# andrewhou1/GeomConsistentFR

Measured on AMD Instinct MI355X. Metric: ray_steps_per_sec, higher is better.
Workload: dtype f64+f32

## Files before the change

### geomconsistentfr_amd/_lib.py

```python
import ctypes
import os

import torch

from . import build as _build

_LIB = None

GCFR_OK = 0
ABI_VERSION = 6
_ERRORS = {-1: "GCFR_ERR_INVALID_ARGUMENT", -2: "GCFR_ERR_LAUNCH"}

_p, _i, _f, _d = ctypes.c_void_p, ctypes.c_int32, ctypes.c_float, ctypes.c_double

N_COUNTERS = 28
COUNTER_NAMES = ("tiles", "groups_nominal", "groups_visited", "bound_tests", "bodies", "lane_samples", "early_exits",
                 "tie_remarches", "samples_in_range", "bounds_given_up", "visits_after_last_body", "visits_before_first_body",
                 "trail_enter", "trail_skips", "trail_leave", "rough_samples", "wave_samples", "wave_samples_taken", "lane_takes",
                 "audit_bound_checks", "audit_bound_violations", "audit_term_checks", "audit_term_violations",
                 "audit_masked_checks", "audit_masked_violations", "audit_safe_violations", "audit_max_use")


class Options(ctypes.Structure):
    _fields_ = [("struct_size", ctypes.c_uint32), ("tile_w", _i), ("group", _i), ("ksplit", _i),
                ("depth_bound_skip", _i), ("lds_stage", _i),
                ("event_start", _p), ("event_stop", _p), ("counters", _p), ("pixels", _i), ("phase", _i)]


def options(tile_w=0, group=0, ksplit=-1, depth_bound_skip=-1, event_start=None,
            event_stop=None, counters=None, lds_stage=-1, pixels=0, phase=0) -> Options:
    o = Options()
    load().gcfr_options_default(ctypes.byref(o))
    o.tile_w, o.group, o.ksplit, o.depth_bound_skip = tile_w, group, ksplit, depth_bound_skip
    o.lds_stage = lds_stage
    o.event_start, o.event_stop, o.counters = event_start, event_stop, counters
    o.pixels = pixels
    o.phase = phase
    return o


def _with(o, field: str, value: int) -> Options:
    n = Options()
    if o is None:
        load().gcfr_options_default(ctypes.byref(n))
    else:
        ctypes.memmove(ctypes.byref(n), ctypes.byref(o), ctypes.sizeof(Options))
    setattr(n, field, value)
    return n


def with_phase(o, phase: int) -> Options:
    return _with(o, "phase", phase)


def with_pixels(o, pixels: int) -> Options:
    return _with(o, "pixels", pixels)


def opt_ref(o):
    return ctypes.byref(o) if o is not None else None


_SIGNATURES = {
    "gcfr_version": (ctypes.c_char_p, []),
    "gcfr_abi_version": (_i, []),
    "gcfr_sample_table": (_i, [_d, _d, _i, _p]),
    "gcfr_light_prep": (_i, [_p, _i, _i, _f, _f, _p, _p, _p]),
    "gcfr_shadow_workspace_bytes": (ctypes.c_size_t, [_i, _i, _i]),
    "gcfr_options_default": (None, [_p]),
    "gcfr_render_from_depth_fwd": (_i, [_p, _i, _f, _f, _p, _p, _i, _d, _d, _d, _d, _f, _i, _p, _p, _i, _i, _i, _i, _i, _p,
                                        _f, _p, _f, _p, _p, _p, _p, _p, _p, _p, _p, _p, _p, ctypes.c_size_t, _p, _p]),
    "gcfr_normals_fwd": (_i, [_p, _i, _i, _i, _d, _d, _d, _d, _f, _i, _p, _p]),
    "gcfr_normals_bwd": (_i, [_p, _p, _i, _i, _i, _d, _d, _d, _d, _f, _i, _p, _p]),
    "gcfr_render_fwd": (_i, [_p, _i, _f, _f, _p, _p, _i, _p, _p, _p, _i, _i, _i, _i, _i, _p, _f, _p, _f,
                             _p, _p, _p, _p, _p, _p, _p, _p, _p, ctypes.c_size_t, _p, _p]),
    "gcfr_shadow_fwd": (_i, [_p, _p, _i, _p, _i, _i, _i, _i, _i, _p, _f, _p, _p, _p, _p, ctypes.c_size_t, _p, _p]),
    "gcfr_shade_fwd": (_i, [_p, _p, _p, _p, _p, _p, _i, _i, _i, _i, _f, _p, _p, _p, _p, _p]),
    "gcfr_shadow_bwd": (_i, [_p, _p, _p, _p, _i, _i, _i, _i, _i, _p, _p, _p, _p]),
    "gcfr_shade_bwd": (_i, [_p, _p, _p, _p, _p, _p, _i, _i, _i, _i, _f, _p, _p, _p, _p, _p, _p, _p, _p, _p, _p, _p]),
    "gcfr_render_bwd": (_i, [_p, _p, _p, _p, _p, _p, _p, _i, _i, _i, _i, _i, _p, _d, _d, _d, _d, _f, _i, _f, _p, _p, _p, _p, _p,
                             _p, _p, _p, _p, _p]),
    "gcfr_light_prep_bwd": (_i, [_p, _i, _i, _f, _f, _p, _p, _p, _p]),
    "gcfr_inference_images_u8": (_i, [_p, _p, _p, _p, _p, _p, _p, _p, _p, _i, _i, _i, _i, _i, _p, _p, _p, _p, _p, _p, _i, _p]),
    "gcfr_fix_border_u8": (_i, [_p, _p, _i, _i, _i, _i, _p, _p]),
    "gcfr_assemble_batch_u8": (_i, [_p, _p, _p, _p, _i, _i, _i, _p, _p, _p, _p, _p]),
    "gcfr_masked_metrics_workspace_bytes": (ctypes.c_size_t, [_i, _i, _i]),
    "gcfr_masked_metrics_u8": (_i, [_p, _p, _p, _i, _i, _i, _i, _p, _p, _p, ctypes.c_size_t, _p]),
    "gcfr_image_losses_workspace_bytes": (ctypes.c_size_t, [_i, _i, _i]),
    "gcfr_image_losses_fwd": (_i, [_p, _p, _p, _i, _i, _i, _i, _p, _d, _p, _p, _p, _p, ctypes.c_size_t, _p]),
    "gcfr_image_losses_bwd": (_i, [_p, _p, _p, _i, _i, _i, _i, _p, _d, _p, _p, _p, _p, _p]),
    "gcfr_supervised_losses_workspace_bytes": (ctypes.c_size_t, [_i, _i, _i]),
    "gcfr_supervised_losses_fwd": (_i, [_p, _p, _p, _p, _p, _p, _p, _p, _p, _p, ctypes.c_int64, _i, _i, _i, _p, _p, _p, ctypes.c_size_t, _p]),
    "gcfr_supervised_losses_bwd": (_i, [_p, _p, _p, _p, _p, _p, _p, _p, _p, ctypes.c_int64, _i, _i, _i, _p, _p, _p, _p, _p, _p, _p, _p,
                                        _p, _p, _p, _p]),
    "gcfr_light_rig_fwd": (_i, [_p, _p, _p, _i, _i, _i, _i, _i, _p, _p, _p]),
    "gcfr_light_rig_bwd": (_i, [_p, _p, _p, _i, _i, _i, _i, _i, _p, _p, _p, _p, _p, _p]),
    "gcfr_light_rig_frames_u8": (_i, [_p, _p, _p, _p, _i, _i, _p, _i, _i, _i, _i, _i, _i, _p, _p]),
    "gcfr_ingest_photographs_u8": (_i, [_p, _i, _i, _i, _i, _p, _p]),
    "gcfr_fullres_composites_u8": (_i, [_p, _p, _p, _p, _i, _i, _i, _i, _i, _i, _f, _f, _p, _p]),
    "gcfr_fullres_composites_guided_u8": (_i, [_p, _p, _p, _p, _i, _i, _i, _i, _i, _i, _f, _f, _f, _p, _p]),
    "gcfr_ingest_box_u8": (_i, [_p, _i, _i, _i, _p, _i, _i, _p, _p]),
    "gcfr_fullres_composites_box_u8": (_i, [_p, _p, _p, _p, _i, _i, _i, _i, _i, _p, _i, _i, _i, _f, _f, _p, _p]),
    "gcfr_fullres_composites_box_guided_u8": (_i, [_p, _p, _p, _p, _i, _i, _i, _i, _i, _p, _i, _i, _i, _f, _f, _f, _p, _p]),
# ... 153 lines not shown
```

### geomconsistentfr_amd/csrc/gcfr_march.hpp

```cpp
#pragma once

#include "gcfr_device.hpp"
#include "gcfr_mutants.hpp"

#include "../../include/gcfr.h"

#include <atomic>
#include <cstddef>
#include <type_traits>

namespace gcfr {

struct ShadowArgs {
    const float *depth;
    const uint8_t *mask;
    const float *light_pt;
    const double *t_table;
    float *min_dist;
    int32_t *argmin;
    int32_t mask_batch, L, H, W, N;
    int32_t tiles_x, tiles_per_image;
    float bonus, bx_lo, bx_hi, by_lo, by_hi;
};

// ... 132 lines not shown
}
__device__ inline float lane_value(float v, int lane)
{
    return __builtin_bit_cast(float, __builtin_amdgcn_readlane(__builtin_bit_cast(int, v), lane));
}


constexpr int kQueueSlot = 64;
enum { kTfOk = 0, kTfStride = 1, kTfTabs = 2, kTfTfirst = 3, kTfInvDt = 4 };
constexpr int kStatChunk = 16384;
__host__ __device__ inline int stat_chunk_shift(int H, int W)
{
    const int raw = (H * W + kStatChunk - 1) >> 14;
    return (raw > 8 && raw <= 16) ? 15 : 14;
}
__host__ __device__ inline int stat_chunk_px(int H, int W) { return 1 << stat_chunk_shift(H, W); }
__host__ __device__ inline int n_stat_chunks(int H, int W)
{
    const int sh = stat_chunk_shift(H, W);
    return (H * W + (1 << sh) - 1) >> sh;
}
static_assert(kStatChunk == 1 << 14, "stat_chunk_shift() spells kStatChunk as a shift");


struct MarchEpilogueArgs {
    float *min_dist;
    int32_t *argmin;
    float bonus, bx_lo, bx_hi, by_lo, by_hi;
    const float *normals;
    const float *albedo;
    const float *ambient;
    float *shadow_w, *full, *final_shading, *rendered;
    float intensity;
    NormalsArgs nrm;
    float *normals_out;
};

struct ShadowQuadArgs {
    const float *depth;
    const float4 *quad;
    const int *bbox;
    const int *diag;
    const float4 *zb;
    const int *zrange;
    const int *mones;
    int *tflag;
    const uint8_t *mask;
    const uint32_t *reserved0;
    const float *light_pt;
    const double *t_table;
    unsigned long long *counters;
    int32_t mask_batch, B, L, H, W, N;
    int32_t tiles_x, tiles_y;
    int32_t bl_offset;
    int32_t hz_off;
    MarchEpilogueArgs epi;
};

typedef const __attribute__((address_space(4))) ShadowQuadArgs *ArgPtr;
typedef const __attribute__((address_space(4))) MarchEpilogueArgs *EpiPtr;
__device__ __forceinline__ ArgPtr kernel_args()
{
    return (ArgPtr)__builtin_amdgcn_kernarg_segment_ptr();
}
template <class T>
__device__ __forceinline__ T launder(T p)
{
    asm volatile("" : "+s"(p));
    return p;
}

constexpr double kRintMagic = 6755399441055744.0;
typedef float f32x4 __attribute__((ext_vector_type(4)));

__device__ inline int lo32(double v)
{
    return (int)(unsigned)(__builtin_bit_cast(unsigned long long, v) & 0xffffffffull);
}

enum { kCntTiles, kCntGroupsNominal, kCntGroupsVisited, kCntBoundTests, kCntBodies, kCntLaneSamples, kCntEarlyExit,
       kCntTieRemarch, kCntSamplesInRange, kCntBoundsGivenUp, kCntVisitsAfterLastBody, kCntVisitsBeforeFirstBody,
       kCntTrailEnter, kCntTrailSkips, kCntTrailLeave, kCntRoughSamples, kCntWaveSamples, kCntWaveSamplesTaken, kCntLaneTakes,
       kCntAuditBoundChecks, kCntAuditBoundViol, kCntAuditTermChecks, kCntAuditTermViol, kCntAuditMaskedChecks, kCntAuditMaskedViol,
       kCntAuditSafeViol, kCntAuditMaxUse, kCntUsed };
static_assert(kCntUsed <= GCFR_N_COUNTERS, "gcfr_options.counters holds GCFR_N_COUNTERS tallies");
#if defined(GCFR_AUDIT) && !defined(GCFR_COUNTERS)
#error "-DGCFR_AUDIT needs -DGCFR_COUNTERS"
#endif
#ifdef GCFR_COUNTERS
#define GCFR_COUNT(i, n) (cnt[i] += (unsigned)(n))
#else
#define GCFR_COUNT(i, n) ((void)0)
#endif

struct ImageStats {
    int r_min, c_min, r_max, c_max;
    int s_min, s_max, d_min, d_max;
    int gz_lo_s, gz_nhi_s;
    int mask_all_ones;
};
__device__ inline ImageStats reduce_image_stats(ArgPtr a, int b, int lane, bool want_z)
{
    const int n = n_stat_chunks(a->H, a->W);
    if (n <= 8) {
        typedef const __attribute__((address_space(4))) int *ConstI32Ptr;
        const ConstI32Ptr sb = (ConstI32Ptr)(unsigned long long)a->bbox + 4 * (size_t)(a->mask_batch == 1 ? 0 : b) * n;
        const ConstI32Ptr sz = (ConstI32Ptr)(unsigned long long)a->zrange + 2 * (size_t)b * n;
        const ConstI32Ptr so = (ConstI32Ptr)(unsigned long long)a->mones + (size_t)(a->mask_batch == 1 ? 0 : b) * n;
        const ConstI32Ptr sd = (ConstI32Ptr)(unsigned long long)a->diag + 4 * (size_t)(a->mask_batch == 1 ? 0 : b) * n;
        int d0 = kBBoxInit, d1 = kBBoxInit, d2 = kBBoxInit, d3 = kBBoxInit;
        int m0 = kBBoxInit, m1 = kBBoxInit, m2 = kBBoxInit, m3 = kBBoxInit, z0 = 0x7fffffff, z1 = 0x7fffffff, ones = 1;
#pragma unroll
        for (int j = 0; j < 8; ++j) {
            if (j < n) {
                m0 = min(m0, sb[4 * j + 0]);
                m1 = min(m1, sb[4 * j + 1]);
                m2 = min(m2, sb[4 * j + 2]);
                m3 = min(m3, sb[4 * j + 3]);
                ones = min(ones, so[j]);
                d0 = min(d0, sd[4 * j + 0]);
                d1 = min(d1, sd[4 * j + 1]);
                d2 = min(d2, sd[4 * j + 2]);
                d3 = min(d3, sd[4 * j + 3]);
                if (want_z) {
                    z0 = min(z0, sz[2 * j + 0]);
                    z1 = min(z1, sz[2 * j + 1]);
                }
            }
        }
        ImageStats st;
        st.r_min = m0;
        st.c_min = m1;
        st.r_max = -m2;
        st.c_max = -m3;
        st.gz_lo_s = z0;
        st.gz_nhi_s = z1;
        st.mask_all_ones = ones;
        st.s_min = d0;
        st.s_max = -d1;
        st.d_min = d2;
        st.d_max = -d3;
        return st;
    }
    const int4 *pb = (const int4 *)a->bbox + (size_t)(a->mask_batch == 1 ? 0 : b) * n;
    const int2 *pz = (const int2 *)a->zrange + (size_t)b * n;
    const int *po = a->mones + (size_t)(a->mask_batch == 1 ? 0 : b) * n;
    const int4 *pd = (const int4 *)a->diag + (size_t)(a->mask_batch == 1 ? 0 : b) * n;
    int4 m = make_int4(kBBoxInit, kBBoxInit, kBBoxInit, kBBoxInit), dg = m;
    int2 mz = make_int2(0x7fffffff, 0x7fffffff);
    int ones = 1;
    for (int j = lane; j < n; j += 64) {
        ones = min(ones, po[j]);
        const int4 v = pb[j];
        m.x = min(m.x, v.x);
        m.y = min(m.y, v.y);
        m.z = min(m.z, v.z);
        m.w = min(m.w, v.w);
        const int4 w = pd[j];
        dg.x = min(dg.x, w.x);
        dg.y = min(dg.y, w.y);
        dg.z = min(dg.z, w.z);
        dg.w = min(dg.w, w.w);
        if (want_z) {
            const int2 vz = pz[j];
            mz.x = min(mz.x, vz.x);
            mz.y = min(mz.y, vz.y);
        }
    }
    ImageStats st;
    st.r_min = wave_min_i32(m.x);
    st.c_min = wave_min_i32(m.y);
    st.r_max = -wave_min_i32(m.z);
    st.c_max = -wave_min_i32(m.w);
    st.gz_lo_s = want_z ? wave_min_i32(mz.x) : 0x7fffffff;
    st.gz_nhi_s = want_z ? wave_min_i32(mz.y) : 0x7fffffff;
    st.mask_all_ones = wave_min_i32(ones);
    st.s_min = wave_min_i32(dg.x);
    st.s_max = -wave_min_i32(dg.y);
    st.d_min = wave_min_i32(dg.z);
    st.d_max = -wave_min_i32(dg.w);
    return st;
}

__device__ inline int fresh_lane_id()
{
    int l;
    asm volatile("v_mbcnt_lo_u32_b32 %0, -1, 0\n\tv_mbcnt_hi_u32_b32 %0, -1, %0" : "=v"(l));
    return l;
}

enum { kModeInline = 0, kModeFull = 1, kModeRough = 2 };
#ifndef GCFR_ROUGH_CHUNK
#define GCFR_ROUGH_CHUNK 3
#endif
#ifndef GCFR_BODY_PIPELINE
#define GCFR_BODY_PIPELINE 1
#endif
#ifndef GCFR_ROUGH_CHUNK_ARGMIN
#define GCFR_ROUGH_CHUNK_ARGMIN 3
#endif
template <int TILE_W, bool EVEN_HALF, bool WANT_ARGMIN, int DEPTH, bool FUSE_SHADE, int SPLIT, bool ALL_ONES = false, bool OWN = false,
          int MODE = kModeInline>
__device__ __forceinline__ bool march_tile(ArgPtr a, const int bl, const int qy, const int tx,
                                           const ImageStats &st)
{
    static_assert(MODE == kModeInline || SPLIT == 0, "full / rough pairs: the grid schedule's kernels");
    constexpr int TILE_H = 64 / TILE_W;
    static_assert(SPLIT == 0 || SPLIT == 1, "SPLIT: 0 = one wave per tile, 1 = the workgroup's four waves split the sample range");
    static_assert(!(OWN && (SPLIT != 0 || ALL_ONES)), "pixels = mask: the grid schedule only");
    const int H = a->H, W = a->W, L = a->L;
    typedef const __attribute__((address_space(4))) double *TablePtr;
    typedef const __attribute__((address_space(4))) float *ConstF32Ptr;
    typedef const __attribute__((address_space(4))) int *ConstI32Ptr;
    const TablePtr tt = (TablePtr)(unsigned long long)a->t_table;
    const int lane = fresh_lane_id();
    const int wave = __builtin_amdgcn_readfirstlane((int)(threadIdx.x >> 6));
    constexpr bool KSPLIT = SPLIT == 1;
    constexpr bool TRAIL = !KSPLIT;
    constexpr bool ROUGH = MODE == kModeRough;
    constexpr bool PIPE = GCFR_BODY_PIPELINE && !WANT_ARGMIN && !KSPLIT && !ROUGH && FUSE_SHADE && DEPTH >= 2;
    const int chunk = KSPLIT ? (a->N + 3) >> 2 : a->N;
    const int k_lo = KSPLIT ? wave * chunk : 0;
    const int N = KSPLIT ? min(a->N, k_lo + chunk) : a->N;
#ifdef GCFR_COUNTERS
    unsigned cnt[kCntUsed] = {};
    unsigned cnt_since_body = 0, cnt_had_body = 0;
    const unsigned long long trace_t0 = __builtin_amdgcn_s_memrealtime(), trace_c0 = __builtin_amdgcn_s_memtime();
#endif

    const int b = bl / L;
    const int l = bl - b * L;
    int r = qy * TILE_H + lane / TILE_W;
    int c = tx * TILE_W + (lane % TILE_W);
    const bool valid = (r < H) && (c < W);
    r = valid ? r : H - 1;
    c = valid ? c : W - 1;

    const size_t P = (size_t)H * W;
    const int Wp = W + 1;
    const size_t Pq = (size_t)(H + 1) * Wp;
    const __amdgpu_buffer_rsrc_t qr = make_rsrc(a->quad + (size_t)b * Pq, (int)(Pq * 16));
    const __amdgpu_buffer_rsrc_t mr =
        make_rsrc(a->mask + (size_t)(a->mask_batch == 1 ? 0 : b) * P, (int)P);

    const bool own_off = GCFR_M(17, false &&, ) OWN && (!valid || (buf_load_u8(mr, __mul24(r, W) + c) == 0));

    const ConstF32Ptr lp = (ConstF32Ptr)(unsigned long long)a->light_pt;
    const float Cx = lp[3 * bl + 0], Cy = lp[3 * bl + 1], Cz = lp[3 * bl + 2];
    const Box box = image_box(H, W);
    const LightCase lc = classify_light(Cx, Cy, box);
    const float halfWf = W / 2.0f, halfHf = H / 2.0f;
    const double halfW = W / 2.0, halfH = H / 2.0;
    const int halfWi = W / 2, halfHi = H / 2;

    const float x = (float)c - halfWf, y = halfHf - (float)r;
    const float zb = a->depth[(size_t)b * P + (size_t)r * W + c];
    float Ex, Ey;
    end_point(x, y, Cx, Cy, box, lc, Ex, Ey);
    const float dxf = Ex - x, dyf = Ey - y;
    const float BCx = Cx - x, BCy = Cy - y, BCz = Cz - zb;
    const bool finite_ray = (dxf - dxf == 0.0f) && (dyf - dyf == 0.0f);
    const double x64 = x, y64 = y;
    const double dx64 = finite_ray ? (double)dxf : 0.0, dy64 = finite_ray ? (double)dyf : 0.0;
    const double Mx = EVEN_HALF ? kRintMagic + halfW : kRintMagic;
    const double My = EVEN_HALF ? kRintMagic + halfH : kRintMagic;
    const int quad_origin = (Wp + 1) << 4;
#ifdef GCFR_AUDIT
    RayConst arc;
    arc.H = H;
    arc.W = W;
    arc.halfW = halfW;
    arc.halfH = halfH;
    arc.x = x;
    arc.y = y;
    arc.zb = zb;
    arc.dx = dxf;
    arc.dy = dyf;
    arc.BCx = BCx;
    arc.BCy = BCy;
    arc.BCz = BCz;
    arc.x64 = x64;
    arc.y64 = y64;
    arc.dx64 = dx64;
    arc.dy64 = dy64;
    const __amdgpu_buffer_rsrc_t azr = make_rsrc(a->depth + (size_t)b * P, (int)(P * 4));
    bool audit_dead = false;
    auto audit_S = [&](int k, bool &masked) -> float {
        const float S = ray_sample(arc, (double)tt[k], azr, mr, masked);
        masked = masked || audit_dead;
        return S;
    };
    auto audit_count = [&](int slot, bool pred) { cnt[slot] += (unsigned)__builtin_popcountll(__builtin_amdgcn_ballot_w64(pred)); };
    auto audit_masked = [&](int k_from, int k_to, bool claim) {
        for (int k = k_from; k < k_to; ++k) {
            bool m;
            (void)audit_S(k, m);
            audit_count(kCntAuditMaskedChecks, claim && finite_ray);
            audit_count(kCntAuditMaskedViol, claim && finite_ray && !m);
        }
    };
#endif
    const ConstI32Ptr tfl = (ConstI32Ptr)(unsigned long long)a->tflag;
    const bool t_increasing = (a->N >= 2) && (tfl[kTfOk] != 0);
    bool use_zb = !ROUGH && (a->zb != nullptr) && t_increasing;
    if (MODE == kModeFull && !use_zb)
        return true;
    const int zrec = tfl[kTfStride];
    const int zls = use_zb ? (zrec & 0xff) : 3;
    const int zntw = (W >> zls) + 1;
    const float nrm = __builtin_amdgcn_sqrtf(BCx * BCx + BCy * BCy);
    const float c1 = BCz * ((dxf * BCx + dyf * BCy) * __builtin_amdgcn_rcpf(nrm));
    const float t_abs = __builtin_bit_cast(float, tfl[kTfTabs]);
#ifndef GCFR_GIVEUP_FACTOR
#define GCFR_GIVEUP_FACTOR 0.5f
// ... 502 lines not shown
                GCFR_COUNT(kCntTrailSkips, 1);
#ifdef GCFR_AUDIT
                audit_safe(cw && !gone);
                audit_masked(k0, min(k0 + DEPTH, k_end), gone);
#endif
#ifdef GCFR_COUNTERS
                ++cnt_since_body;
#endif
                if (check_hz) {
                    float dxl, dyl;
                    dir_f32(dxl, dyl);
                    const int ci = (int)__builtin_floorf(__builtin_fmaf(tn, dxl, x)), ri = (int)__builtin_floorf(-__builtin_fmaf(tn, dyl, y));
                    constexpr int C = kHorizonDim / 2, M = kHorizonDim - 1;
                    const int ic = (dxl >= 0.0f) ? kHorizonDim + min(max(ci + C, 0), M) : min(max(ci + C, 0), M);
                    const int ir = (dyl > 0.0f) ? 2 * kHorizonDim + min(max(ri + C, 0), M) : 3 * kHorizonDim + min(max(ri + C, 0), M);
                    const f32x4 zc4 = __builtin_bit_cast(f32x4, __builtin_amdgcn_raw_buffer_load_b128(zr, hz_off + (ic << 4), 0, 0));
                    const f32x4 zr4 = __builtin_bit_cast(f32x4, __builtin_amdgcn_raw_buffer_load_b128(zr, hz_off + (ir << 4), 0, 0));
                    const float zc = fmaxf(fmaxf(zc4.x, zc4.y), fmaxf(zc4.z, zc4.w)), zr_ = fmaxf(fmaxf(zr4.x, zr4.y), fmaxf(zr4.z, zr4.w));
                    float nrm_l = nrm;
                    asm volatile("" : "+v"(nrm_l));
                    const float Dc = __builtin_fmaf(nrm_l, fminf(zc, zr_), -(nrm_l * zb)) + Kerr;
                    const float gd = __builtin_fmaf(c1, tn, -Dc);
                    const bool past = lane_last < k0 + DEPTH GCFR_M(26, + 1, );
                    const bool finished = (GCFR_M(11, true, (c1 > 0.0f)) && (gd > 0.0f) && (gd * gd * GCFR_M(8, GCFR_MUT_SLACK_VALUE, 0.998f) > bestS) && (bestS < safeS)) || past;
                    if (__builtin_amdgcn_ballot_w64(!finished) == 0ull) {
                        any_masked |= past;
                        GCFR_COUNT(kCntEarlyExit, 1);
#ifdef GCFR_AUDIT
                        audit_finish(k0 + DEPTH, GCFR_M(11, true, (c1 > 0.0f)) && (gd > 0.0f) && (gd * gd * GCFR_M(8, GCFR_MUT_SLACK_VALUE, 0.998f) > bestS) && (bestS < safeS),
                                     gd, GCFR_M(8, GCFR_MUT_SLACK_VALUE, 0.998f), past);
#endif
                        break;
                    }
                } else if (!finish_check(k0, tc0, check)) {
                    break;
                }
            } else {
                GCFR_COUNT(kCntTrailLeave, 1);
                uint32_t cm[DEPTH];
#pragma unroll
                for (int j = 0; j < DEPTH; ++j) {
                    const double tj = (j == 0) ? ta64 : ((j == DEPTH - 1) ? tb64 : (double)tt[clampk(k0 + j)]);
                    int cj, rj;
                    cm[j] = ALL_ONES ? 1u : buf_load_u8(mr, mask_offset(x64 + tj * dx64, y64 + tj * dy64, cj, rj));
                }
                if (!consume(k0, cm, zcur, ta64, tb64, tc0, check, std::true_type{}, cw, []() {}))
                    break;
                zcur = record_of(tc0, tc3);
                continue;
            }
            zcur = znext;
        }
    }
    }

    if (KSPLIT) {
        __shared__ float sS[4][64], sPS[4][64];
        __shared__ int sK[4][64], sPK[4][64];
        __shared__ uint8_t sM[4][64];
        sS[wave][lane] = bestS;
        sK[wave][lane] = besti;
        sPS[wave][lane] = prevS;
        sPK[wave][lane] = prevk;
        sM[wave][lane] = any_masked ? 1 : 0;
        __syncthreads();
        if (wave != 0)
            return false;
#pragma unroll
        for (int q = 1; q < 4; ++q) {
            const float Sq = sS[q][lane];
            const bool take = Sq < bestS;
            const float PSq = sPS[q][lane];
            const bool local_pred = PSq < bestS;
            prevS = take ? (local_pred ? PSq : bestS) : prevS;
            prevk = take ? (local_pred ? sPK[q][lane] : besti) : prevk;
            bestS = take ? Sq : bestS;
            besti = take ? sK[q][lane] : besti;
            any_masked |= (sM[q][lane] != 0);
        }
    }

    float BCx_e = BCx;
    asm volatile("" : "+v"(BCx_e));
    const int lane_e = fresh_lane_id();
    const int r_e = qy * TILE_H + lane_e / TILE_W, c_e = tx * TILE_W + (lane_e % TILE_W);
    const bool valid_e = (r_e < H) && (c_e < W);
    r = valid_e ? r_e : H - 1;
    c = valid_e ? c_e : W - 1;
    const size_t pix = (size_t)r * W + c;
    const size_t o = (size_t)bl * P + pix;
    const EpiPtr ep = launder((EpiPtr)&a->epi);
    float *const min_dist = ep->min_dist;
    int32_t *const argmin = WANT_ARGMIN ? ep->argmin : nullptr;
    const float bonus = ep->bonus, bx_lo = ep->bx_lo, bx_hi = ep->bx_hi, by_lo = ep->by_lo, by_hi = ep->by_hi;
    const float *const normals = FUSE_SHADE ? ep->normals : nullptr;
    const float *const albedo = FUSE_SHADE ? ep->albedo : nullptr;
    float *const shadow_w = FUSE_SHADE ? ep->shadow_w : nullptr, *const full = FUSE_SHADE ? ep->full : nullptr;
    float *const final_shading = FUSE_SHADE ? ep->final_shading : nullptr, *const rendered = FUSE_SHADE ? ep->rendered : nullptr;
    float *const normals_out = FUSE_SHADE ? ep->normals_out : nullptr;
    const float intensity = FUSE_SHADE ? ep->intensity : 0.0f;
    const float amb = FUSE_SHADE ? ((ConstF32Ptr)(unsigned long long)ep->ambient)[bl] : 0.0f;
    NormalsArgs na = {};
    float zs[9], n[3], alb[3];
    if (FUSE_SHADE) {
        na.H = H;
        na.W = W;
        na.inv_fx = ep->nrm.inv_fx;
        na.inv_fy = ep->nrm.inv_fy;
        na.cx = ep->nrm.cx;
        na.cy = ep->nrm.cy;
        na.z_offset = ep->nrm.z_offset;
        na.negate_y = ep->nrm.negate_y;
        if (normals) {
            const float *nrm_in = normals + (size_t)b * 3 * P + pix;
            n[0] = nrm_in[0];
            n[1] = nrm_in[P];
            n[2] = nrm_in[2 * P];
        } else {
            load_depth_stencil(H, W, a->depth + (size_t)b * P, r, c, zs);
        }
        const float *alb_in = albedo + (size_t)b * 3 * P + pix;
#pragma unroll
        for (int ch = 0; ch < 3; ++ch)
            alb[ch] = alb_in[ch * P];
    }

    const float den = sqrt_rn_normal(((BCx_e * BCx_e + BCy * BCy) + BCz * BCz) + kEps4);
    float d = sqrt_rn_normal(bestS) / den;
    if (WANT_ARGMIN) {
        const bool tie = GCFR_M(16, false &&, ) (prevk >= 0) && (sqrt_rn_normal(prevS) / den == d);
        if (__builtin_amdgcn_ballot_w64(tie) != 0ull) {
            GCFR_COUNT(kCntTieRemarch, 1);
            RayConst rc;
            rc.H = H;
            rc.W = W;
            rc.halfW = halfW;
            rc.halfH = halfH;
            rc.x = x;
            rc.y = y;
            rc.zb = zb;
            dir_f32(rc.dx, rc.dy);
            rc.BCx = BCx;
            rc.BCy = BCy;
            rc.BCz = BCz;
            rc.x64 = x64;
            rc.y64 = y64;
            rc.dx64 = dx64;
            rc.dy64 = dy64;
            const int first = first_tied_sample(rc, a->t_table, make_rsrc(a->depth + (size_t)b * P, (int)(P * 4)), mr,
                                                tie, prevk, den, d);
            besti = tie ? first : besti;
        }
    }
    if (any_masked && !(d < kMaskedDistance)) {
        d = kMaskedDistance;
        besti = -1;
    }
    if (OWN && (lane_last < 0)) {
        d = kMaskedDistance;
        besti = -1;
    }
    if (!finite_ray)
        d = __builtin_nanf("");
    const bool inside = (Cx >= bx_lo) && (Cx <= bx_hi) && (Cy >= by_lo) && (Cy <= by_hi);
    if (inside)
        d = d + bonus;
    if (!valid_e)
        return false;
    auto store = [](auto *p, auto v) {
        if (!WANT_ARGMIN)
            __builtin_nontemporal_store(v, p);
        else
            *p = v;
    };
    store(min_dist + o, d);
    if (WANT_ARGMIN)
        store(argmin + o, besti);
    if (FUSE_SHADE) {
        if (!normals) {
            unit_normal_from(na, zs, r, c, n);
            if (normals_out && l == 0) {
                float *no = normals_out + (size_t)b * 3 * P + pix;
                store(no, n[0]);
                store(no + P, n[1]);
                store(no + 2 * P, n[2]);
            }
        }
        const Shaded sh = shade_pixel(x, y, zb, n[0], n[1], n[2], Cx, Cy, Cz, amb, intensity, d);
        if (shadow_w)
            store(shadow_w + o, sh.w);
        if (full)
            store(full + o, sh.full);
        if (final_shading)
            store(final_shading + o, sh.fin);
        float *ren = rendered + (size_t)bl * 3 * P + pix;
#pragma unroll
        for (int ch = 0; ch < 3; ++ch)
            store(ren + ch * P, alb[ch] * sh.fin);
    }
#ifdef GCFR_COUNTERS
    if (a->counters && lane == 0 && !(KSPLIT && wave != 0)) {
        cnt[kCntVisitsAfterLastBody] += cnt_since_body;
#ifndef GCFR_TRACE_ONLY
#pragma unroll
        for (int i = 0; i < kCntUsed; ++i) {
            if (i == kCntAuditMaxUse)
                atomicMax(a->counters + i, (unsigned long long)cnt[i]);
            else
                atomicAdd(a->counters + i, (unsigned long long)cnt[i]);
        }
#endif
        unsigned long long *rec = a->counters + GCFR_N_COUNTERS + 4 * ((size_t)(bl * a->tiles_y + qy) * a->tiles_x + tx);
        const unsigned hw_id = __builtin_amdgcn_s_getreg((31 << 11) | 4);
        const unsigned xcc_id = __builtin_amdgcn_s_getreg((31 << 11) | 20);
        rec[0] = trace_t0;
        rec[1] = __builtin_amdgcn_s_memrealtime();
        rec[2] = __builtin_amdgcn_s_memtime() - trace_c0;
        rec[3] = (unsigned long long)hw_id | ((unsigned long long)(xcc_id & 0xf) << 32) |
                 ((unsigned long long)(cnt[kCntBodies] & 0xfff) << 36) | ((unsigned long long)(cnt[kCntGroupsVisited] & 0xfff) << 48);
    }
#endif
    return false;
}

#ifndef GCFR_MARCH_WAVES_PER_EU
#define GCFR_MARCH_WAVES_PER_EU 6
#endif
#ifndef GCFR_MARCH_ARGMIN_WAVES_PER_EU
#define GCFR_MARCH_ARGMIN_WAVES_PER_EU 5
#endif

template <int TILE_W, bool EVEN_HALF, bool WANT_ARGMIN, int DEPTH, bool FUSE_SHADE, bool OWN = false>
__device__ __forceinline__ void march_grid(ArgPtr a)
{
    const int wave = __builtin_amdgcn_readfirstlane((int)(threadIdx.x >> 6));
    const int tx = (int)blockIdx.x * 4 + wave;
    const int bl = a->bl_offset + (int)blockIdx.z;
    const bool want_z = (a->zb != nullptr);
    const ImageStats st = reduce_image_stats(a, bl / a->L, threadIdx.x & 63, want_z);
    if (tx >= a->tiles_x)
        return;
    bool rough;
    if (st.mask_all_ones != 0)
        rough = march_tile<TILE_W, EVEN_HALF, WANT_ARGMIN, DEPTH, FUSE_SHADE, 0, true, false, kModeFull>(a, bl, (int)blockIdx.y, tx, st);
    else
        rough = march_tile<TILE_W, EVEN_HALF, WANT_ARGMIN, DEPTH, FUSE_SHADE, 0, false, OWN, kModeFull>(a, bl, (int)blockIdx.y, tx, st);
    if (GCFR_M(15, false &&, ) __builtin_amdgcn_readfirstlane((int)rough) != 0) {
        const ArgPtr a2 = WANT_ARGMIN ? a : launder(a);
        const int bl2 = WANT_ARGMIN ? bl : a2->bl_offset + (int)blockIdx.z;
        const ImageStats st2 = WANT_ARGMIN ? st : reduce_image_stats(a2, bl2 / a2->L, threadIdx.x & 63, false);
        if (st2.mask_all_ones != 0)
            march_tile<TILE_W, EVEN_HALF, WANT_ARGMIN, DEPTH, FUSE_SHADE, 0, true, false, kModeRough>(a2, bl2, (int)blockIdx.y, tx, st2);
        else
            march_tile<TILE_W, EVEN_HALF, WANT_ARGMIN, DEPTH, FUSE_SHADE, 0, false, OWN, kModeRough>(a2, bl2, (int)blockIdx.y, tx, st2);
    }
}

enum { kSchedGrid = 0 };

template <int SCHED, int TILE_W, bool EVEN_HALF, bool WANT_ARGMIN, int DEPTH, bool FUSE_SHADE, bool OWN = false>
__device__ __forceinline__ void march_dispatch()
{
    static_assert(SCHED == kSchedGrid, "the product library has the grid schedule only");
    march_grid<TILE_W, EVEN_HALF, WANT_ARGMIN, DEPTH, FUSE_SHADE, OWN>(kernel_args());
}

template <int TILE_W, bool EVEN_HALF, int DEPTH, bool FUSE_SHADE, int SCHED>
__global__ __launch_bounds__(256)
__attribute__((amdgpu_waves_per_eu(GCFR_MARCH_WAVES_PER_EU, GCFR_MARCH_WAVES_PER_EU))) void shadow_fwd_quad_kernel(ShadowQuadArgs)
{
    march_dispatch<SCHED, TILE_W, EVEN_HALF, false, DEPTH, FUSE_SHADE>();
}
template <int TILE_W, bool EVEN_HALF, int DEPTH, bool FUSE_SHADE, int SCHED>
__global__ __launch_bounds__(256)
__attribute__((amdgpu_waves_per_eu(GCFR_MARCH_ARGMIN_WAVES_PER_EU, GCFR_MARCH_ARGMIN_WAVES_PER_EU))) void shadow_fwd_quad_argmin_kernel(ShadowQuadArgs)
{
    march_dispatch<SCHED, TILE_W, EVEN_HALF, true, DEPTH, FUSE_SHADE>();
}
template <int TILE_W, bool EVEN_HALF, int DEPTH, bool FUSE_SHADE, int SCHED>
__global__ __launch_bounds__(256)
__attribute__((amdgpu_waves_per_eu(GCFR_MARCH_ARGMIN_WAVES_PER_EU, GCFR_MARCH_ARGMIN_WAVES_PER_EU))) void shadow_fwd_quad_argmin_own_kernel(ShadowQuadArgs)
{
    march_dispatch<SCHED, TILE_W, EVEN_HALF, true, DEPTH, FUSE_SHADE, true>();
}
template <int TILE_W, bool EVEN_HALF, bool WANT_ARGMIN, int DEPTH, bool FUSE_SHADE>
__global__ __launch_bounds__(256) void shadow_fwd_quad_ksplit_kernel(ShadowQuadArgs)
{
    const ArgPtr a = kernel_args();
    const int bl = a->bl_offset + (int)blockIdx.z;
    const ImageStats st = reduce_image_stats(a, bl / a->L, threadIdx.x & 63, a->zb != nullptr);
    march_tile<TILE_W, EVEN_HALF, WANT_ARGMIN, DEPTH, FUSE_SHADE, 1>(a, bl, (int)blockIdx.y, (int)blockIdx.x, st);
}


enum Schedule { kGrid = kSchedGrid, kKSplit, kGridOwn };

template <int TILE_W, int DEPTH, bool FUSE>
static void launch_quad4(const ShadowQuadArgs &a, bool even_half, bool want_argmin, Schedule sch, dim3 grid, hipStream_t st)
{
#define GCFR_LAUNCH(KERNEL, ...) hipLaunchKernelGGL((KERNEL<TILE_W, __VA_ARGS__>), grid, dim3(256), 0, st, a)
    if (sch == kKSplit) {
        if (even_half) {
            if (want_argmin)
                GCFR_LAUNCH(shadow_fwd_quad_ksplit_kernel, true, true, DEPTH, FUSE);
            else
                GCFR_LAUNCH(shadow_fwd_quad_ksplit_kernel, true, false, DEPTH, FUSE);
        } else {
            if (want_argmin)
                GCFR_LAUNCH(shadow_fwd_quad_ksplit_kernel, false, true, DEPTH, FUSE);
            else
                GCFR_LAUNCH(shadow_fwd_quad_ksplit_kernel, false, false, DEPTH, FUSE);
        }
    } else if (sch == kGridOwn) {
        if (even_half)
            GCFR_LAUNCH(shadow_fwd_quad_argmin_own_kernel, true, DEPTH, FUSE, kSchedGrid);
        else
            GCFR_LAUNCH(shadow_fwd_quad_argmin_own_kernel, false, DEPTH, FUSE, kSchedGrid);
    } else {
        if (even_half) {
            if (want_argmin)
                GCFR_LAUNCH(shadow_fwd_quad_argmin_kernel, true, DEPTH, FUSE, kSchedGrid);
            else
                GCFR_LAUNCH(shadow_fwd_quad_kernel, true, DEPTH, FUSE, kSchedGrid);
        } else {
            if (want_argmin)
                GCFR_LAUNCH(shadow_fwd_quad_argmin_kernel, false, DEPTH, FUSE, kSchedGrid);
            else
                GCFR_LAUNCH(shadow_fwd_quad_kernel, false, DEPTH, FUSE, kSchedGrid);
        }
    }
#undef GCFR_LAUNCH
}

template <int TILE_W, int DEPTH>
static void launch_quad3(const ShadowQuadArgs &a, bool even_half, bool want_argmin, Schedule sch, dim3 grid, hipStream_t st)
{
    if (a.epi.rendered)
        launch_quad4<TILE_W, DEPTH, true>(a, even_half, want_argmin, sch, grid, st);
    else
        launch_quad4<TILE_W, DEPTH, false>(a, even_half, want_argmin, sch, grid, st);
}

typedef void (*MarchUnitFn)(const ShadowQuadArgs &a, bool even_half, bool want_argmin, Schedule sch, dim3 grid, hipStream_t st);
#define GCFR_MARCH_UNIT_NAME_(TW, G) launch_march_##TW##_##G
#define GCFR_MARCH_UNIT_NAME(TW, G) GCFR_MARCH_UNIT_NAME_(TW, G)
#define GCFR_DECLARE_MARCH_UNIT(TW, G)                                                                              \
    void GCFR_MARCH_UNIT_NAME(TW, G)(const ShadowQuadArgs &a, bool even_half, bool want_argmin, Schedule sch, dim3 grid, \
                                     hipStream_t st);
GCFR_DECLARE_MARCH_UNIT(16, 4)
#ifndef GCFR_FAST_BUILD
GCFR_DECLARE_MARCH_UNIT(16, 2)
GCFR_DECLARE_MARCH_UNIT(16, 1)
GCFR_DECLARE_MARCH_UNIT(8, 4)
GCFR_DECLARE_MARCH_UNIT(8, 2)
GCFR_DECLARE_MARCH_UNIT(8, 1)
GCFR_DECLARE_MARCH_UNIT(32, 4)
GCFR_DECLARE_MARCH_UNIT(32, 2)
GCFR_DECLARE_MARCH_UNIT(32, 1)
GCFR_DECLARE_MARCH_UNIT(64, 4)
GCFR_DECLARE_MARCH_UNIT(64, 2)
GCFR_DECLARE_MARCH_UNIT(64, 1)
#endif

}
```

### geomconsistentfr_amd/csrc/gcfr_mutants.hpp

```cpp
#pragma once

#ifndef GCFR_MUT
#define GCFR_MUT 0
#endif

#ifndef GCFR_MUT_SLACK_VALUE
#define GCFR_MUT_SLACK_VALUE 1.002f
#endif
#define GCFR_PP_CAT_(a, b, c) a##b##_##c
#define GCFR_PP_CAT(a, b, c) GCFR_PP_CAT_(a, b, c)
#define GCFR_PP_SECOND_(a, b, ...) b
#define GCFR_PP_SECOND(...) GCFR_PP_SECOND_(__VA_ARGS__)
#define GCFR_PP_IS_PAIR(x) GCFR_PP_SECOND(x, 0, ~)
#define GCFR_PP_IF_0(mut, prod) prod
#define GCFR_PP_IF_1(mut, prod) mut
#define GCFR_PP_IF_(c) GCFR_PP_IF_##c
#define GCFR_PP_IF(c) GCFR_PP_IF_(c)
#define GCFR_M(n, mut, prod) GCFR_PP_IF(GCFR_PP_IS_PAIR(GCFR_PP_CAT(GCFR_MUT_PAIR_, GCFR_MUT, n)))(mut, prod)

#define GCFR_MUT_PAIR_1_1 ~, 1
#define GCFR_MUT_PAIR_2_2 ~, 1
#define GCFR_MUT_PAIR_3_3 ~, 1
#define GCFR_MUT_PAIR_4_4 ~, 1
#define GCFR_MUT_PAIR_5_5 ~, 1
#define GCFR_MUT_PAIR_6_6 ~, 1
#define GCFR_MUT_PAIR_7_7 ~, 1
#define GCFR_MUT_PAIR_8_8 ~, 1
#define GCFR_MUT_PAIR_9_9 ~, 1
#define GCFR_MUT_PAIR_10_10 ~, 1
#define GCFR_MUT_PAIR_11_11 ~, 1
#define GCFR_MUT_PAIR_13_13 ~, 1
#define GCFR_MUT_PAIR_14_14 ~, 1
#define GCFR_MUT_PAIR_15_15 ~, 1
#define GCFR_MUT_PAIR_16_16 ~, 1
#define GCFR_MUT_PAIR_17_17 ~, 1
#define GCFR_MUT_PAIR_18_18 ~, 1
#define GCFR_MUT_PAIR_20_20 ~, 1
#define GCFR_MUT_PAIR_21_21 ~, 1
#define GCFR_MUT_PAIR_22_22 ~, 1
#define GCFR_MUT_PAIR_23_23 ~, 1
#define GCFR_MUT_PAIR_24_24 ~, 1
#define GCFR_MUT_PAIR_25_25 ~, 1
#define GCFR_MUT_PAIR_26_26 ~, 1
#define GCFR_MUT_PAIR_27_27 ~, 1
#define GCFR_MUT_PAIR_29_29 ~, 1
```

Measured before the change: 2507 billion.

## Skip marching tiles whose rays provably cannot reach any unmasked pixel

```diff
diff --git a/geomconsistentfr_amd/_lib.py b/geomconsistentfr_amd/_lib.py
--- a/geomconsistentfr_amd/_lib.py
+++ b/geomconsistentfr_amd/_lib.py
@@ -18,7 +18,8 @@
                  "tie_remarches", "samples_in_range", "bounds_given_up", "visits_after_last_body", "visits_before_first_body",
                  "trail_enter", "trail_skips", "trail_leave", "rough_samples", "wave_samples", "wave_samples_taken", "lane_takes",
                  "audit_bound_checks", "audit_bound_violations", "audit_term_checks", "audit_term_violations",
-                 "audit_masked_checks", "audit_masked_violations", "audit_safe_violations", "audit_max_use")
+                 "audit_masked_checks", "audit_masked_violations", "audit_safe_violations", "audit_max_use",
+                 "tiles_unreachable")
 
 
 class Options(ctypes.Structure):
diff --git a/geomconsistentfr_amd/csrc/gcfr_march.hpp b/geomconsistentfr_amd/csrc/gcfr_march.hpp
--- a/geomconsistentfr_amd/csrc/gcfr_march.hpp
+++ b/geomconsistentfr_amd/csrc/gcfr_march.hpp
@@ -238,7 +238,8 @@
        kCntTieRemarch, kCntSamplesInRange, kCntBoundsGivenUp, kCntVisitsAfterLastBody, kCntVisitsBeforeFirstBody,
        kCntTrailEnter, kCntTrailSkips, kCntTrailLeave, kCntRoughSamples, kCntWaveSamples, kCntWaveSamplesTaken, kCntLaneTakes,
        kCntAuditBoundChecks, kCntAuditBoundViol, kCntAuditTermChecks, kCntAuditTermViol, kCntAuditMaskedChecks, kCntAuditMaskedViol,
-       kCntAuditSafeViol, kCntAuditMaxUse, kCntUsed };
+       kCntAuditSafeViol, kCntAuditMaxUse,
+       kCntTilesUnreachable, kCntUsed };
 static_assert(kCntUsed <= GCFR_N_COUNTERS, "gcfr_options.counters holds GCFR_N_COUNTERS tallies");
 #if defined(GCFR_AUDIT) && !defined(GCFR_COUNTERS)
 #error "-DGCFR_AUDIT needs -DGCFR_COUNTERS"
@@ -345,6 +346,59 @@
     return l;
 }
 
+constexpr float kReachMaxLight = 1048576.0f;
+template <int TILE_W, int TILE_H>
+__device__ inline bool tile_unreachable(int H, int W, int qy, int tx, float Cx, float Cy, const LightCase &lc, const ImageStats &st)
+{
+    asm volatile("" : "+s"(H), "+s"(W));
+    if (!((fabsf(Cx) <= kReachMaxLight) && (fabsf(Cy) <= kReachMaxLight)) || (max(H, W) > 4096))
+        return false;
+    const int c0 = tx * TILE_W, c1 = min(c0 + TILE_W, W) - 1, r0 = qy * TILE_H, r1 = min(r0 + TILE_H, H) - 1;
+    const int PXa = 2 * c0 - W, PXb = 2 * c1 - W, PYa = H - 2 * r1, PYb = H - 2 * r0;
+    const int CXa = __builtin_amdgcn_readfirstlane((int)__builtin_floorf(2.0f * Cx)), CXb = __builtin_amdgcn_readfirstlane((int)__builtin_ceilf(2.0f * Cx));
+    const int CYa = __builtin_amdgcn_readfirstlane((int)__builtin_floorf(2.0f * Cy)), CYb = __builtin_amdgcn_readfirstlane((int)__builtin_ceilf(2.0f * Cy));
+    const int EXa = max(min(PXa, CXa), -W), EXb = min(max(PXb, CXb), W - 2);
+    const int EYa = max(min(PYa, CYa), 2 - H), EYb = min(max(PYb, CYb), H);
+    bool apart = st.r_min == kBBoxInit;
+    if (!apart) {
+        const int mx = GCFR_M(30, 0, 2), md = GCFR_M(30, 0, 3);
+        const int SXa = min(PXa, EXa), SXb = max(PXb, EXb), SYa = min(PYa, EYa), SYb = max(PYb, EYb);
+        const int SUa = min(PXa - PYb, EXa - EYb), SUb = max(PXb - PYa, EXb - EYa);
+        const int SVa = min(PXa + PYa, EXa + EYa), SVb = max(PXb + PYb, EXb + EYb);
+        const int ws = W + H, wd = W - H;
+        apart = (SXb + mx <= 2 * st.c_min - W) || (SXa - mx >= 2 * st.c_max - W) ||
+                (SYb + mx <= H - 2 * st.r_max) || (SYa - mx >= H - 2 * st.r_min) ||
+                (SUb + md <= 2 * st.s_min - ws) || (SUa - md >= 2 * st.s_max - ws) ||
+                (SVb + md <= 2 * st.d_min - wd) || (SVa - md >= 2 * st.d_max - wd);
+    }
+    if (!apart)
+        return false;
+    if ((lc.xcase == 1) && (lc.ycase == 1))
+        return true;
+    const float xa = 0.5f * (float)PXa, xb = 0.5f * (float)PXb, ya = 0.5f * (float)PYa, yb = 0.5f * (float)PYb;
+    const float dx_min = fmaxf(fmaxf(xa - Cx, Cx - xb), 0.0f), dx_max = fmaxf(fabsf(Cx - xa), fabsf(Cx - xb));
+    const float dy_min = fmaxf(fmaxf(ya - Cy, Cy - yb), 0.0f), dy_max = fmaxf(fabsf(Cy - ya), fabsf(Cy - yb));
+    if (!(dx_min >= 1.0f))
+        return false;
+    const float inv_dx_min = __builtin_amdgcn_rcpf(dx_min);
+    const float m_max = 1.001f * dy_max * inv_dx_min;
+    const float M = m_max * (fabsf(Cx) + (float)W) + fabsf(Cy) + (float)H;
+    float delta = 2.0e-3f + 1.1e-4f * m_max + 6.0e-7f * M;
+    if (!((lc.xcase != 1) && (lc.ycase == 1))) {
+        const float m_lo = 0.999f * dy_min * __builtin_amdgcn_rcpf(dx_max + 1.0e-4f) - 1.0e-4f;
+        if (!(m_lo >= 4.0e-4f))
+            return false;
+        const float rho = 1.1e-4f * inv_dx_min + 3.0e-7f;
+        delta += ((0.75f * (float)W + 1.0f) * 1.0e-4f + 6.0e-7f * M) * __builtin_amdgcn_rcpf(m_lo) +
+                 1.01f * rho * (fabsf(Cx) + 0.5f * (float)W + 1.0f);
+    }
+    return delta <= 0.2f;
+}
+
+template <int TILE_W, bool WANT_ARGMIN, bool FUSE_SHADE, class Distance, class Pixel, class Tally>
+__device__ __forceinline__ void tile_epilogue(Distance distance, Pixel pixel, Tally tally, const ArgPtr a, const int bl, const int b, const int qy,
+                                              const int tx, const float Cx, const float Cy, const float Cz);
+
 enum { kModeInline = 0, kModeFull = 1, kModeRough = 2 };
 #ifndef GCFR_ROUGH_CHUNK
 #define GCFR_ROUGH_CHUNK 3
@@ -385,7 +439,6 @@
 #endif
 
     const int b = bl / L;
-    const int l = bl - b * L;
     int r = qy * TILE_H + lane / TILE_W;
     int c = tx * TILE_W + (lane % TILE_W);
     const bool valid = (r < H) && (c < W);
@@ -1054,12 +1107,93 @@
 
     float BCx_e = BCx;
     asm volatile("" : "+v"(BCx_e));
+    tile_epilogue<TILE_W, WANT_ARGMIN, FUSE_SHADE>([&](float &d_out, int &besti_out) {
+    const float den = sqrt_rn_normal(((BCx_e * BCx_e + BCy * BCy) + BCz * BCz) + kEps4);
+    float d = sqrt_rn_normal(bestS) / den;
+    if (WANT_ARGMIN) {
+        const bool tie = GCFR_M(16, false &&, ) (prevk >= 0) && (sqrt_rn_normal(prevS) / den == d);
+        if (__builtin_amdgcn_ballot_w64(tie) != 0ull) {
+            GCFR_COUNT(kCntTieRemarch, 1);
+            RayConst rc;
+            rc.H = H;
+            rc.W = W;
+            rc.halfW = halfW;
+            rc.halfH = halfH;
+            rc.x = x;
+            rc.y = y;
+            rc.zb = zb;
+            dir_f32(rc.dx, rc.dy);
+            rc.BCx = BCx;
+            rc.BCy = BCy;
+            rc.BCz = BCz;
+            rc.x64 = x64;
+            rc.y64 = y64;
+            rc.dx64 = dx64;
+            rc.dy64 = dy64;
+            const int first = first_tied_sample(rc, a->t_table, make_rsrc(a->depth + (size_t)b * P, (int)(P * 4)), mr,
+                                                tie, prevk, den, d);
+            besti = tie ? first : besti;
+        }
+    }
+    if (any_masked && !(d < kMaskedDistance)) {
+        d = kMaskedDistance;
+        besti = -1;
+    }
+    if (OWN && (lane_last < 0)) {
+        d = kMaskedDistance;
+        besti = -1;
+    }
+    if (!finite_ray)
+        d = __builtin_nanf("");
+    d_out = d;
+    besti_out = besti;
+    }, [&](int, int, float &x_, float &y_, float &zb_) {
+        x_ = x;
+        y_ = y;
+        zb_ = zb;
+    }, [&]() {
+#ifdef GCFR_COUNTERS
+    if (a->counters && lane == 0 && !(KSPLIT && wave != 0)) {
+        cnt[kCntVisitsAfterLastBody] += cnt_since_body;
+#ifndef GCFR_TRACE_ONLY
+#pragma unroll
+        for (int i = 0; i < kCntUsed; ++i) {
+            if (i == kCntAuditMaxUse)
+                atomicMax(a->counters + i, (unsigned long long)cnt[i]);
+            else
+                atomicAdd(a->counters + i, (unsigned long long)cnt[i]);
+        }
+#endif
+        unsigned long long *rec = a->counters + GCFR_N_COUNTERS + 4 * ((size_t)(bl * a->tiles_y + qy) * a->tiles_x + tx);
+        const unsigned hw_id = __builtin_amdgcn_s_getreg((31 << 11) | 4);
+        const unsigned xcc_id = __builtin_amdgcn_s_getreg((31 << 11) | 20);
+        rec[0] = trace_t0;
+        rec[1] = __builtin_amdgcn_s_memrealtime();
+        rec[2] = __builtin_amdgcn_s_memtime() - trace_c0;
+        rec[3] = (unsigned long long)hw_id | ((unsigned long long)(xcc_id & 0xf) << 32) |
+                 ((unsigned long long)(cnt[kCntBodies] & 0xfff) << 36) | ((unsigned long long)(cnt[kCntGroupsVisited] & 0xfff) << 48);
+    }
+#endif
+    }, a, bl, b, qy, tx, Cx, Cy, Cz);
+    return false;
+}
+
+template <int TILE_W, bool WANT_ARGMIN, bool FUSE_SHADE, class Distance, class Pixel, class Tally>
+__device__ __forceinline__ void tile_epilogue(Distance distance, Pixel pixel, Tally tally, const ArgPtr a, const int bl, const int b, const int qy,
+                                              const int tx, const float Cx, const float Cy, const float Cz)
+{
+    constexpr int TILE_H = 64 / TILE_W;
+    typedef const __attribute__((address_space(4))) float *ConstF32Ptr;
+    const int H = a->H, W = a->W;
+    const int l = bl - b * a->L;
+    const size_t P = (size_t)H * W;
     const int lane_e = fresh_lane_id();
     const int r_e = qy * TILE_H + lane_e / TILE_W, c_e = tx * TILE_W + (lane_e % TILE_W);
     const bool valid_e = (r_e < H) && (c_e < W);
-    r = valid_e ? r_e : H - 1;
-    c = valid_e ? c_e : W - 1;
+    const int r = valid_e ? r_e : H - 1, c = valid_e ? c_e : W - 1;
     const size_t pix = (size_t)r * W + c;
+    float x, y, zb;
+    pixel(r, c, x, y, zb);
     const size_t o = (size_t)bl * P + pix;
     const EpiPtr ep = launder((EpiPtr)&a->epi);
     float *const min_dist = ep->min_dist;
@@ -1097,48 +1231,14 @@
             alb[ch] = alb_in[ch * P];
     }
 
-    const float den = sqrt_rn_normal(((BCx_e * BCx_e + BCy * BCy) + BCz * BCz) + kEps4);
-    float d = sqrt_rn_normal(bestS) / den;
-    if (WANT_ARGMIN) {
-        const bool tie = GCFR_M(16, false &&, ) (prevk >= 0) && (sqrt_rn_normal(prevS) / den == d);
-        if (__builtin_amdgcn_ballot_w64(tie) != 0ull) {
-            GCFR_COUNT(kCntTieRemarch, 1);
-            RayConst rc;
-            rc.H = H;
-            rc.W = W;
-            rc.halfW = halfW;
-            rc.halfH = halfH;
-            rc.x = x;
-            rc.y = y;
-            rc.zb = zb;
-            dir_f32(rc.dx, rc.dy);
-            rc.BCx = BCx;
-            rc.BCy = BCy;
-            rc.BCz = BCz;
-            rc.x64 = x64;
-            rc.y64 = y64;
-            rc.dx64 = dx64;
-            rc.dy64 = dy64;
-            const int first = first_tied_sample(rc, a->t_table, make_rsrc(a->depth + (size_t)b * P, (int)(P * 4)), mr,
-                                                tie, prevk, den, d);
-            besti = tie ? first : besti;
-        }
-    }
-    if (any_masked && !(d < kMaskedDistance)) {
-        d = kMaskedDistance;
-        besti = -1;
-    }
-    if (OWN && (lane_last < 0)) {
-        d = kMaskedDistance;
-        besti = -1;
-    }
-    if (!finite_ray)
-        d = __builtin_nanf("");
+    float d;
+    int besti_e;
+    distance(d, besti_e);
     const bool inside = (Cx >= bx_lo) && (Cx <= bx_hi) && (Cy >= by_lo) && (Cy <= by_hi);
     if (inside)
         d = d + bonus;
     if (!valid_e)
-        return false;
+        return;
     auto store = [](auto *p, auto v) {
         if (!WANT_ARGMIN)
             __builtin_nontemporal_store(v, p);
@@ -1147,7 +1247,7 @@
     };
     store(min_dist + o, d);
     if (WANT_ARGMIN)
-        store(argmin + o, besti);
+        store(argmin + o, besti_e);
     if (FUSE_SHADE) {
         if (!normals) {
             unit_normal_from(na, zs, r, c, n);
@@ -1170,29 +1270,108 @@
         for (int ch = 0; ch < 3; ++ch)
             store(ren + ch * P, alb[ch] * sh.fin);
     }
+    tally();
+}
+
+template <int TILE_W>
+__device__ inline bool tile_skips_march(ArgPtr a, int bl, int qy, int tx, const ImageStats &st)
+{
+    typedef const __attribute__((address_space(4))) float *ConstF32Ptr;
+    typedef const __attribute__((address_space(4))) int *ConstI32Ptr;
+    if ((st.mask_all_ones != 0) || (a->N < 2) || (((ConstI32Ptr)(unsigned long long)a->tflag)[kTfOk] == 0))
+        return false;
+    const ConstF32Ptr lp = (ConstF32Ptr)(unsigned long long)a->light_pt;
+    const float Cx = lp[3 * bl + 0], Cy = lp[3 * bl + 1];
+    const LightCase lc = classify_light(Cx, Cy, image_box(a->H, a->W));
+    return tile_unreachable<TILE_W, 64 / TILE_W>(a->H, a->W, qy, tx, Cx, Cy, lc, st);
+}
+
+template <int TILE_W, bool WANT_ARGMIN, int DEPTH, bool FUSE_SHADE>
+__device__ __forceinline__ void skipped_tile(ArgPtr a, const int bl, const int qy, const int tx, const bool lead)
+{
+    typedef const __attribute__((address_space(4))) float *ConstF32Ptr;
+    if (!lead)
+        return;
+    const int H = a->H, W = a->W;
+    const int b = bl / a->L;
+    const ConstF32Ptr lp = (ConstF32Ptr)(unsigned long long)a->light_pt;
+    const float Cx = lp[3 * bl + 0], Cy = lp[3 * bl + 1], Cz = lp[3 * bl + 2];
 #ifdef GCFR_COUNTERS
-    if (a->counters && lane == 0 && !(KSPLIT && wave != 0)) {
-        cnt[kCntVisitsAfterLastBody] += cnt_since_body;
+    const unsigned long long trace_t0 = __builtin_amdgcn_s_memrealtime(), trace_c0 = __builtin_amdgcn_s_memtime();
+    unsigned audit_checks = 0, audit_viol = 0;
+#endif
+#ifdef GCFR_AUDIT
+    {
+        constexpr int TILE_H = 64 / TILE_W;
+        const int lane = fresh_lane_id();
+        const int r0 = qy * TILE_H + lane / TILE_W, c0 = tx * TILE_W + (lane % TILE_W);
+        const bool valid = (r0 < H) && (c0 < W);
+        const int r = valid ? r0 : H - 1, c = valid ? c0 : W - 1;
+        const size_t P = (size_t)H * W;
+        const Box box = image_box(H, W);
+        RayConst arc;
+        arc.H = H;
+        arc.W = W;
+        arc.halfW = W / 2.0;
+        arc.halfH = H / 2.0;
+        arc.x = (float)c - W / 2.0f;
+        arc.y = H / 2.0f - (float)r;
+        arc.zb = a->depth[(size_t)b * P + (size_t)r * W + c];
+        float Ex, Ey;
+        end_point(arc.x, arc.y, Cx, Cy, box, classify_light(Cx, Cy, box), Ex, Ey);
+        arc.dx = Ex - arc.x;
+        arc.dy = Ey - arc.y;
+        const bool finite_ray = (arc.dx - arc.dx == 0.0f) && (arc.dy - arc.dy == 0.0f);
+        arc.BCx = Cx - arc.x;
+        arc.BCy = Cy - arc.y;
+        arc.BCz = Cz - arc.zb;
+        arc.x64 = arc.x;
+        arc.y64 = arc.y;
+        arc.dx64 = finite_ray ? (double)arc.dx : 0.0;
+        arc.dy64 = finite_ray ? (double)arc.dy : 0.0;
+        const __amdgpu_buffer_rsrc_t azr = make_rsrc(a->depth + (size_t)b * P, (int)(P * 4));
+        const __amdgpu_buffer_rsrc_t amr = make_rsrc(a->mask + (size_t)(a->mask_batch == 1 ? 0 : b) * P, (int)P);
+        auto count = [](bool pred) { return (unsigned)__builtin_popcountll(__builtin_amdgcn_ballot_w64(pred)); };
+        audit_checks += count(valid);
+        audit_viol += count(valid && !finite_ray);
+        for (int k = 0; k < a->N; ++k) {
+            bool m;
+            (void)ray_sample(arc, a->t_table[k], azr, amr, m);
+            audit_checks += count(valid && finite_ray);
+            audit_viol += count(valid && finite_ray && !m);
+        }
+    }
+#endif
+    tile_epilogue<TILE_W, WANT_ARGMIN, FUSE_SHADE>(
+        [](float &d, int &besti) {
+            d = kMaskedDistance;
+            besti = -1;
+        },
+        [&](int r, int c, float &x, float &y, float &zb) {
+            x = (float)c - W / 2.0f;
+            y = H / 2.0f - (float)r;
+            zb = a->depth[(size_t)b * ((size_t)H * W) + (size_t)r * W + c];
+        },
+        [&]() {
+#ifdef GCFR_COUNTERS
+            if (a->counters && fresh_lane_id() == 0) {
 #ifndef GCFR_TRACE_ONLY
-#pragma unroll
-        for (int i = 0; i < kCntUsed; ++i) {
-            if (i == kCntAuditMaxUse)
-                atomicMax(a->counters + i, (unsigned long long)cnt[i]);
-            else
-                atomicAdd(a->counters + i, (unsigned long long)cnt[i]);
-        }
-#endif
-        unsigned long long *rec = a->counters + GCFR_N_COUNTERS + 4 * ((size_t)(bl * a->tiles_y + qy) * a->tiles_x + tx);
-        const unsigned hw_id = __builtin_amdgcn_s_getreg((31 << 11) | 4);
-        const unsigned xcc_id = __builtin_amdgcn_s_getreg((31 << 11) | 20);
-        rec[0] = trace_t0;
-        rec[1] = __builtin_amdgcn_s_memrealtime();
-        rec[2] = __builtin_amdgcn_s_memtime() - trace_c0;
-        rec[3] = (unsigned long long)hw_id | ((unsigned long long)(xcc_id & 0xf) << 32) |
-                 ((unsigned long long)(cnt[kCntBodies] & 0xfff) << 36) | ((unsigned long long)(cnt[kCntGroupsVisited] & 0xfff) << 48);
-    }
-#endif
-    return false;
+                atomicAdd(a->counters + kCntTiles, 1ull);
+                atomicAdd(a->counters + kCntTilesUnreachable, 1ull);
+                atomicAdd(a->counters + kCntGroupsNominal, (unsigned long long)((a->N + DEPTH - 1) / DEPTH));
+                atomicAdd(a->counters + kCntAuditMaskedChecks, (unsigned long long)audit_checks);
+                atomicAdd(a->counters + kCntAuditMaskedViol, (unsigned long long)audit_viol);
+#endif
+                unsigned long long *rec = a->counters + GCFR_N_COUNTERS + 4 * ((size_t)(bl * a->tiles_y + qy) * a->tiles_x + tx);
+                rec[0] = trace_t0;
+                rec[1] = __builtin_amdgcn_s_memrealtime();
+                rec[2] = __builtin_amdgcn_s_memtime() - trace_c0;
+                rec[3] = (unsigned long long)__builtin_amdgcn_s_getreg((31 << 11) | 4) |
+                         ((unsigned long long)(__builtin_amdgcn_s_getreg((31 << 11) | 20) & 0xf) << 32);
+            }
+#endif
+        },
+        a, bl, b, qy, tx, Cx, Cy, Cz);
 }
 
 #ifndef GCFR_MARCH_WAVES_PER_EU
@@ -1212,6 +1391,10 @@
     const ImageStats st = reduce_image_stats(a, bl / a->L, threadIdx.x & 63, want_z);
     if (tx >= a->tiles_x)
         return;
+    if (__builtin_amdgcn_readfirstlane((int)tile_skips_march<TILE_W>(a, bl, (int)blockIdx.y, tx, st)) != 0) {
+        skipped_tile<TILE_W, WANT_ARGMIN, DEPTH, FUSE_SHADE>(a, bl, (int)blockIdx.y, tx, true);
+        __builtin_amdgcn_endpgm();
+    }
     bool rough;
     if (st.mask_all_ones != 0)
         rough = march_tile<TILE_W, EVEN_HALF, WANT_ARGMIN, DEPTH, FUSE_SHADE, 0, true, false, kModeFull>(a, bl, (int)blockIdx.y, tx, st);
@@ -1261,7 +1444,10 @@
     const ArgPtr a = kernel_args();
     const int bl = a->bl_offset + (int)blockIdx.z;
     const ImageStats st = reduce_image_stats(a, bl / a->L, threadIdx.x & 63, a->zb != nullptr);
-    march_tile<TILE_W, EVEN_HALF, WANT_ARGMIN, DEPTH, FUSE_SHADE, 1>(a, bl, (int)blockIdx.y, (int)blockIdx.x, st);
+    if (__builtin_amdgcn_readfirstlane((int)tile_skips_march<TILE_W>(a, bl, (int)blockIdx.y, (int)blockIdx.x, st)) == 0)
+        march_tile<TILE_W, EVEN_HALF, WANT_ARGMIN, DEPTH, FUSE_SHADE, 1>(a, bl, (int)blockIdx.y, (int)blockIdx.x, st);
+    else
+        skipped_tile<TILE_W, WANT_ARGMIN, DEPTH, FUSE_SHADE>(a, bl, (int)blockIdx.y, (int)blockIdx.x, __builtin_amdgcn_readfirstlane((int)(threadIdx.x >> 6)) == 0);
 }
 
 
diff --git a/geomconsistentfr_amd/csrc/gcfr_mutants.hpp b/geomconsistentfr_amd/csrc/gcfr_mutants.hpp
--- a/geomconsistentfr_amd/csrc/gcfr_mutants.hpp
+++ b/geomconsistentfr_amd/csrc/gcfr_mutants.hpp
@@ -44,3 +44,4 @@
 #define GCFR_MUT_PAIR_26_26 ~, 1
 #define GCFR_MUT_PAIR_27_27 ~, 1
 #define GCFR_MUT_PAIR_29_29 ~, 1
+#define GCFR_MUT_PAIR_30_30 ~, 1
```

After: 2466 billion. 1.7% lower.
